# JGCRI/xanthos

Measured on AMD Instinct MI355X. Metric: cell-months/sec (pm_abcd_mrtm, 67,420 cells), higher is better.
Workload: dtype f64

## Files before the change

### xanthos_amd/csrc/xh_mrtm_wave_launch.hip

```cpp
#include <algorithm>
#include "xh_mrtm_wave_unit.h"
#undef A

namespace {

__global__ void k_mrtm_wave_args(WaveArgs a, WaveArgs *dst, uint4 *cnt, unsigned cnt_vec) {
    if (threadIdx.x == 0) *dst = a;
    if (threadIdx.x == 0 && a.months_ready)
        __hip_atomic_store(const_cast<unsigned *>(a.months_ready), a.ready_at_launch, __ATOMIC_RELAXED, __HIP_MEMORY_SCOPE_AGENT);
    for (unsigned i = threadIdx.x; i < cnt_vec; i += blockDim.x) cnt[i] = make_uint4(0u, 0u, 0u, 0u);
}

}

int wave_launch(xh_ctx *ctx, FlowPlan *fp, const FlowSched &s, const FlowIO &io, hipStream_t st, unsigned **place) {
    if (!fp || fp->n_units == 0) return XH_OK;
    if (!fp->skew_ok || fp->max_imports > 8 * SK_R || fp->max_exports > 8 * SK_R || s.ntmin < fp->skew_lmax + 2 * GROUP) {
        if (xh_flow_debug())
            fprintf(stderr, "time-skewed kernel not used: skew_ok %d, imports %d, outlets %d, shortest month %d sub-steps, largest lag %d\n",
                    (int)fp->skew_ok, fp->max_imports, fp->max_exports, s.ntmin, fp->skew_lmax);
        return XH_ERR_LIMIT;
    }
    {
        uint64_t limit = (uint64_t)1 << 32;
        if (const char *env = getenv("XH_WAVE_ROW_LIMIT")) limit = std::min<uint64_t>(limit, strtoull(env, nullptr, 10));
        const uint64_t stride = io.feed ? 128u : (uint64_t)s.nmonths * 8u;
        if ((uint64_t)(fp->max_cell + 1) * stride > limit || (io.feed && (int64_t)fp->max_cell >= io.feed->ncell)) {
            if (xh_flow_debug())
                fprintf(stderr, "round-3 time-skewed kernel not used: %d rows x %d months x 8 B exceed its 32-bit row offsets\n",
                        fp->max_cell + 1, s.nmonths);
            return XH_ERR_LIMIT;
        }
    }
    int rs = 2048;
    while (rs < 8 * CH + 4 * fp->skew_lmax || rs < 1024 + (2 * CH + 256) * fp->skew_span) rs *= 2;
    if (const char *env = getenv("XH_FLOW_RS")) {
        const int v = atoi(env);
        if (v >= 2048 && (v & (v - 1)) == 0) rs = v;
    }
    const size_t x_streams = (size_t)std::max(fp->n_edges, 1) * (size_t)rs * sizeof(v2d);
    if (x_streams + (size_t)rs * 16 > ((size_t)1 << 32)) return XH_ERR_LIMIT;
    const size_t x_cnt = ((size_t)(fp->n_edges + fp->n_units + PLACE_WORDS) * sizeof(unsigned) + 255) & ~size_t(255);
    const size_t x_rec0 = ((size_t)(s.nit + 3) * sizeof(MonthRec) + 255) & ~size_t(255);
    const size_t x_rec = x_rec0 + (((size_t)(s.nit + 2) * sizeof(FinRec) + 255) & ~size_t(255));
    if (x_streams + x_cnt + x_rec > fp->x_bytes) {
        if (fp->d_x) {
            XH_HIP(ctx, hipStreamSynchronize(st));
            XH_HIP(ctx, hipFree(fp->d_x));
            fp->d_x = nullptr;
        }
        XH_HIP(ctx, hipMalloc(&fp->d_x, x_streams + x_cnt + x_rec));
        fp->x_bytes = x_streams + x_cnt + x_rec;
        fp->rec_key = 0;
    }
    unsigned *cnt = reinterpret_cast<unsigned *>(static_cast<char *>(fp->d_x) + x_streams);
    MonthRec *d_rec = reinterpret_cast<MonthRec *>(static_cast<char *>(fp->d_x) + x_streams + x_cnt);
    FinRec *d_fin = reinterpret_cast<FinRec *>(static_cast<char *>(fp->d_x) + x_streams + x_cnt + x_rec0);
    const FlowFeed *feed = io.feed;
    auto q_off = [&](int m) -> long long {
        if (!feed) return (long long)m * 8;
        return (long long)(m >> 4) * feed->ncell * 128 + (long long)(m & 15) * 8;
    };
    uint64_t rec_key = XH_FNV_BASIS;
    {
        const long long lay[4] = {s.nit, s.total, feed ? (long long)feed->ncell : -1ll, (long long)(size_t)fp->d_x};
        rec_key = xh_fnv1a(rec_key, lay, sizeof(lay));
        rec_key = xh_fnv1a(rec_key, s.h_m, sizeof(int) * (size_t)s.nit);
        rec_key = xh_fnv1a(rec_key, s.h_nt, sizeof(int) * (size_t)s.nit);
        rec_key = xh_fnv1a(rec_key, s.h_g, sizeof(int) * (size_t)(s.nit + 1));
        rec_key = xh_fnv1a(rec_key, s.h_wr, (size_t)s.nit);
        rec_key = xh_fnv1a(rec_key, s.h_secs, sizeof(double) * (size_t)s.nit);
        if (rec_key == 0) rec_key = 1;
    }
    if (rec_key != fp->rec_key) {
        fp->rec_key = 0;
        fp->h_rec.assign((size_t)(s.nit + 3) * sizeof(MonthRec), 0);
        MonthRec *h = reinterpret_cast<MonthRec *>(fp->h_rec.data());
        for (int it = 0; it < s.nit; ++it) {
            h[it].m = s.h_m[it];
            h[it].nt = s.h_nt[it];
            h[it].g = s.h_g[it];
            h[it].write = s.h_wr[it];
            h[it].secs = s.h_secs[it];
            h[it].q_off = q_off(s.h_m[it]);
        }
        h[s.nit].g = s.total;
        fp->h_fin.assign((size_t)(s.nit + 2) * sizeof(FinRec), 0);
        FinRec *hf = reinterpret_cast<FinRec *>(fp->h_fin.data());
        for (int it = 0; it <= s.nit; ++it) {
            if (it >= 1) {
                hf[it].m_prev_w = h[it - 1].m | (h[it - 1].write ? FIN_WRITE : 0);
                hf[it].nt_prev = h[it - 1].nt;
            }
            hf[it].nt_prev = std::max(hf[it].nt_prev, 1);
            hf[it].secs_next1 = it + 1 < s.nit ? h[it + 1].secs : 1.0;
            hf[it].m_next2 = it + 2 < s.nit ? h[it + 2].m : 0;
            hf[it].q_off_next2 = q_off(hf[it].m_next2);
            hf[it].g_next1 = it + 1 <= s.nit ? h[it + 1].g : s.total;
        }
        hf[s.nit + 1].nt_prev = 1;
        hf[s.nit + 1].secs_next1 = 1.0;
        XH_HIP(ctx, hipMemcpyAsync(d_rec, h, fp->h_rec.size(), hipMemcpyHostToDevice, st));
        XH_HIP(ctx, hipMemcpyAsync(d_fin, hf, fp->h_fin.size(), hipMemcpyHostToDevice, st));
        fp->rec_key = rec_key;
    }

    const int cus = ctx->prop.multiProcessorCount > 0 ? ctx->prop.multiProcessorCount : 256;
    const void *kernel = fp->rsum ? wave_rsum_kernel() : wave_exact_kernel();
    const size_t lds_static = (size_t)RING * NSLOT * sizeof(v2d) + LANES * sizeof(uint2) + 2 * LANES * sizeof(unsigned) +
                              LANES * sizeof(double) + 64 +
                              (fp->rsum ? 2 * LANES * sizeof(unsigned) + LANES * sizeof(double) : 0);
    int n_excl = 0;
    if (fp->rsum && fp->n_special >= 0 && fp->n_pair_units > 0 && xh_env_on("XH_RSUM_EXCL", true))
        n_excl = std::min(fp->n_pair_units, 0xffff);
    int n_wg = 0, resident = 0;
    size_t lds = 0;
    {
        n_wg = fp->n_units + cus;
        if (n_wg > 8 * cus) n_wg = std::max(fp->n_units, 8 * cus);
        {
            const char *env = getenv("XH_FLOW_SPARE");
            if (env) n_wg = fp->n_units + std::max(atoi(env), 0);
        }
        const int per_cu = (n_wg + cus - 1) / cus + 3;
        const size_t share = ((size_t)(160 * 1024) / (size_t)per_cu) & ~size_t(1023);
        lds = share > lds_static + 1024 ? share - lds_static : 0;
        XH_HIP(ctx, hipFuncSetAttribute(kernel, hipFuncAttributeMaxDynamicSharedMemorySize, (int)lds));
        XH_HIP(ctx, hipOccupancyMaxActiveBlocksPerMultiprocessor(&resident, kernel, LANES, lds));
        if ((int64_t)(resident - 1) * cus < n_wg || n_wg > 8 * cus) return XH_ERR_LIMIT;
    }

    WaveArgs a;
    a.cell_of_slot = static_cast<const int *>(fp->d_cell_of_slot.p);
    a.lag = static_cast<const int *>(fp->d_lag.p);
    a.ghost_lag = static_cast<const int *>(fp->d_ghost_lag.p);
    a.export_edge = static_cast<const int *>(fp->d_export_edge.p);
    a.ghost_edge = static_cast<const int *>(fp->d_ghost_edge.p);
    a.edge_cons_unit = static_cast<const int *>(fp->d_edge_cons_unit.p);
    a.ent2 = static_cast<const unsigned *>(fp->d_ent2.p);
    a.eprev = static_cast<const unsigned *>(fp->d_eprev.p);
    a.unit_p = static_cast<const int *>(fp->d_unit_p.p);
    a.unit_order = static_cast<const int *>(fp->d_unit_order.p);
    a.n_units = fp->n_units;
    a.unit_lmax = static_cast<const int *>(fp->d_unit_lmax.p);
    a.unit_glmax = static_cast<const int *>(fp->d_unit_glmax.p);
    a.total_slots = (int64_t)fp->n_units * LANES;
    a.nmonths = s.nmonths;
    a.nit = s.nit;
    a.total = s.total;
    a.odd_ok = s.nt_even ? 0 : 1;
    a.rec = d_rec;
    a.fin = d_fin;
    a.lane_flags = static_cast<const unsigned char *>(fp->d_lane_flags.p);
    a.dt = s.dt;
    a.dtinv = 1.0 / s.dt;
    a.flow_dist = io.flow_dist;
    a.velocity = io.velocity;
    a.area = io.area;
    a.runoff = feed ? feed->q_staged : io.runoff;
    a.q_row_stride = feed ? 128u : (unsigned)s.nmonths * 8u;
    a.ready_at_launch = feed ? feed->ready_at_launch : UINT_MAX;
    a.months_ready = feed ? feed->months_ready : nullptr;
    a.place_epoch = feed ? feed->place_epoch : nullptr;
    a.epoch = feed ? feed->epoch : 0u;
    a.n_excl = n_excl;
    a.fenced = xh_env_on("XH_ROUTE_FENCED", false) ? 1 : 0;
    a.S0 = io.S0;
    a.chs = io.chs;
    a.avg = io.avg;
    a.S_end = io.S_end;
    a.F_end = io.F_end;
    a.xbuf = static_cast<char *>(fp->d_x);
    a.xbytes = (unsigned)x_streams;
    a.ring_mask_b = (unsigned)rs * 16u - 1u;
    a.rs = rs;
    a.ready = cnt;
    a.done = cnt + fp->n_edges;
    a.place = cnt + fp->n_edges + fp->n_units;
    *place = a.place;
    unsigned *fault = nullptr;
    int rc = xh_fault_word(ctx, &fault);
    if (rc) return rc;
    a.fault = fault;
    if (s.test_fault) XH_HIP(ctx, hipMemsetD32Async(reinterpret_cast<hipDeviceptr_t>(fault), (int)FAULT_TEST, 1, st));
    a.stats = nullptr;
    {
        const char *env = getenv("XH_FLOW_STATS");
        if (env && env[0] == '1') {
            if (!fp->d_stats) XH_HIP(ctx, hipMalloc(reinterpret_cast<void **>(&fp->d_stats), (size_t)fp->n_units * 48));
            a.stats = fp->d_stats;
        }
    }
    a.fold_cell = static_cast<const int *>(fp->d_fold_cell.p);
    if (!fp->d_skew_args) XH_HIP(ctx, hipMalloc(&fp->d_skew_args, sizeof(WaveArgs) + 256));
    hipLaunchKernelGGL(k_mrtm_wave_args, dim3(1), dim3(256), 0, st, a, static_cast<WaveArgs *>(fp->d_skew_args),
                       reinterpret_cast<uint4 *>(cnt), (unsigned)(x_cnt / sizeof(uint4)));
    {
        const WaveArgs *d_args = static_cast<const WaveArgs *>(fp->d_skew_args);
        void *kargs[] = {&d_args};
        XH_HIP(ctx, hipLaunchKernel(kernel, dim3((unsigned)n_wg), dim3(LANES), kargs, lds, st));
    }
    XH_HIP(ctx, hipGetLastError());
    return XH_OK;
}
```

### xanthos_amd/csrc/xh_mrtm_wave_unit.h

```cpp
#pragma once
#include <algorithm>
#include <climits>
#include <cstdlib>
#include <type_traits>

#include "xh_mrtm_flow.h"

namespace {


constexpr int LANES = 64;
constexpr int SK_P = 4;
#ifndef XH_WAVE_MIDZONE
#define XH_WAVE_MIDZONE 1
#endif
#ifndef XH_WAVE_BMOV
#define XH_WAVE_BMOV 1
#endif
constexpr int NSLOT = 2 * LANES + 1;
constexpr int RING = 8;
constexpr int GROUP = 16;
constexpr int SK_R = 2;
#ifndef XH_WAVE_CH
#define XH_WAVE_CH 256
#endif
constexpr int CH = XH_WAVE_CH;
constexpr unsigned FAULT_DATA_WAIT = 1, FAULT_RING_WAIT = 2, FAULT_PLACE_WAIT = 3, FAULT_GUARD = XH_FAULT_GUARD;
constexpr unsigned FAULT_TEST = 99;
constexpr int PLACE_KEYS = 16 * 8 * 2 * 16 * 4;

constexpr int PLACE_WORDS = 16 + PLACE_KEYS + PLACE_KEYS / 4;

struct MonthRec {
    int m, nt, g, write;
    double secs;
    long long q_off;
};
static_assert(sizeof(MonthRec) == 32, "MonthRec is read with one s_load_dwordx8");

struct FinRec {
    int m_prev_w, nt_prev;
    int m_next2;
    int g_next1;
    double secs_next1;
    long long q_off_next2;
};
constexpr int FIN_WRITE = 1 << 30;
static_assert(sizeof(FinRec) == 32, "FinRec is read with one s_load_dwordx8");

struct WaveArgs {
    const int *cell_of_slot, *lag, *ghost_lag, *export_edge, *ghost_edge, *edge_cons_unit;
    const unsigned *ent2;
    const unsigned *eprev;
    const int *unit_p, *unit_lmax, *unit_glmax;
    const unsigned char *lane_flags;
    int64_t total_slots;
    int nmonths, nit, total;
    const int *unit_order;
    unsigned *place;
    int n_units;
    int odd_ok;
    const MonthRec *rec;
    const FinRec *fin;
    double dt, dtinv;
    const double *flow_dist, *velocity, *area, *runoff, *S0;
    double *chs, *avg, *S_end, *F_end;
    unsigned q_row_stride;
    unsigned ready_at_launch;
    const unsigned *months_ready;
    unsigned *place_epoch;
    unsigned epoch;
    int n_excl;
    int fenced;
    char *xbuf;
    unsigned xbytes;
    unsigned ring_mask_b;
    int rs;
    unsigned *ready;
    unsigned *done;
    unsigned *fault;
    unsigned long long *stats;
    const int *fold_cell;
};

__device__ __forceinline__ unsigned ld_relaxed(const unsigned *p) {
    return __hip_atomic_load(p, __ATOMIC_RELAXED, __HIP_MEMORY_SCOPE_AGENT);
}

constexpr unsigned long long SPIN_LIMIT_TICKS = 500000000ull;

__device__ __forceinline__ bool wave_wait_ge(bool need, const unsigned *p, unsigned target, unsigned &seen,
                                             unsigned *fault, unsigned code) {
    bool ok = !need || seen >= target;
    if (__all(ok)) return true;
    const unsigned long long t0 = __builtin_amdgcn_s_memrealtime();
    for (;;) {
        if (!ok) {
            seen = ld_relaxed(p);
            ok = seen >= target;
        }
        if (__all(ok)) return true;
        if (ld_relaxed(fault) != 0) return false;
        if (__builtin_amdgcn_s_memrealtime() - t0 > SPIN_LIMIT_TICKS) {
            __hip_atomic_store(fault, code, __ATOMIC_RELAXED, __HIP_MEMORY_SCOPE_AGENT);
            return false;
        }
        __builtin_amdgcn_s_sleep(4);
    }
}

typedef double v2d __attribute__((ext_vector_type(2)));
typedef unsigned v4u __attribute__((ext_vector_type(4)));
constexpr int AUX_SC1 = 16;
typedef __attribute__((address_space(3))) const char lds_cchar;
typedef __attribute__((address_space(3))) char lds_char;

typedef __attribute__((address_space(4))) const WaveArgs WaveArgsK;
template <class T>
__device__ __forceinline__ T xh_ldarg(__attribute__((address_space(4))) const T *p) {
    asm volatile("" : "+s"(p));
    return *p;
}
#define A(f) xh_ldarg(&ap->f)

template <bool ONE> struct Val;
template <> struct Val<false> {
    typedef v2d T;
    typedef __attribute__((address_space(3))) const v2d lds_c;
    typedef __attribute__((address_space(3))) v2d lds_m;
    static constexpr unsigned B = 16;
    static __device__ __forceinline__ T zero() { return v2d{0.0, 0.0}; }
};
template <> struct Val<true> {
    typedef double T;
    typedef __attribute__((address_space(3))) const double lds_c;
    typedef __attribute__((address_space(3))) double lds_m;
    static constexpr unsigned B = 8;
    static __device__ __forceinline__ T zero() { return 0.0; }
};

template <int PRE, int POST, int NG, bool CHAIN, bool RSUM = false, bool FOLD = false, int SGL = 0, int NXR = -1>
__device__ __forceinline__ void wave_unit(WaveArgsK *ap, char *lds_generic, uint2 *xtab,
                                          __attribute__((address_space(3))) unsigned *qstage,
                                          __attribute__((address_space(3))) double *fend, const int unit) {
    constexpr bool HAS_G = NG > 0;
    constexpr bool V8 = SGL == 1;
    typedef Val<V8> V;
    typedef typename V::T val_t;
    typedef typename V::lds_c lds_cv;
    typedef typename V::lds_m lds_mv;
    constexpr unsigned VB = V::B;
    constexpr unsigned SLOTB = NSLOT * VB;
    lds_char *lds0 = (lds_char *)lds_generic;
    const int lane = threadIdx.x;
    const int64_t slot = (int64_t)unit * LANES + lane;

    const int gc = A(cell_of_slot)[slot];
    const bool valid = gc >= 0;
    const int gc_safe = valid ? gc : 0;
    const unsigned row_off = (unsigned)gc_safe * A(q_row_stride);
    const double tauinv = valid ? A(velocity)[gc] / A(flow_dist)[gc] : 0.0;
    const double acoef = 1.0 - tauinv * A(dt);
    const double area = valid ? A(area)[gc] : 0.0;
    const double S0v = (valid && A(S0)) ? A(S0)[gc] : 0.0;
    auto ent_off = [](unsigned o) { return V8 ? o >> 1 : o; };
    static_assert(!RSUM || (PRE <= 1 && POST == 0), "reassociated form: one inflow entry");
    static_assert(!FOLD || (RSUM && NG == 0), "folded leaves: reassociated form, units without imports");
    static_assert(SGL == 0 || RSUM, "single-sum plans: reassociated form");
    const int gcL = FOLD ? A(fold_cell)[slot] : -1;
    const bool validL = FOLD && valid && gcL >= 0;
    const unsigned row_offL = (unsigned)(validL ? gcL : 0) * A(q_row_stride);
    const double tauL = validL ? A(velocity)[gcL] / A(flow_dist)[gcL] : 0.0;
    const double acoefL = 1.0 - tauL * A(dt);
    const double areaL = validL ? A(area)[gcL] : 0.0;
    const double S0L = (validL && A(S0)) ? A(S0)[gcL] : 0.0;
    double SL = 0.0, favgL = 0.0, erlL = 0.0, erlL_n = 0.0, snapSL = 0.0, snapAL = 0.0, FL = 0.0;
    constexpr double FOLD_EPS = 1e-6;
    unsigned gfold = (validL && !(tauL * A(dt) <= 1.0 - 1.0 / 1048576.0 && tauL >= 0.0 && S0L >= 0.0)) ? 1u : 0u;
    constexpr double SGL_EPS = 1e-6;
    constexpr double SGL_XEPS = 1e-10;
    unsigned gsgl = 0;
    bool xlane = false;
    double fmin_seen = 0.0;
    if (SGL != 0) {
        const unsigned lf = A(lane_flags)[slot];
        xlane = valid && (lf & 2u) != 0;
        gsgl = (valid && (!(tauinv >= 0.0) || (!(tauinv * A(dt) <= 1.0 - 1.0 / 1048576.0) && !(lf & 1u)) || S0v < 0.0)) ? 1u : 0u;
    }
    constexpr int PRE_N = PRE > 0 ? PRE : 1, POST_N = POST > 0 ? POST : 1;
    lds_cchar *epre[PRE_N], *epost[POST_N];
#pragma unroll
    for (int w = 0; w < PRE; ++w) epre[w] = lds0 + ent_off(A(ent2)[(int64_t)w * A(total_slots) + slot]);
#pragma unroll
    for (int w = 0; w < POST; ++w) epost[w] = lds0 + ent_off(A(ent2)[(int64_t)(SK_P + w) * A(total_slots) + slot]);
    lds_cchar *eprv = lds0 + (CHAIN ? ent_off(A(eprev)[slot]) : 0u);
    lds_mv *own = (lds_mv *)lds0 + lane;
    const int xedge = A(export_edge)[slot];
    const int gedge = A(ghost_edge)[slot];
    const bool has_x = xedge >= 0, has_g = gedge >= 0;
    const unsigned long long xmask = __ballot(has_x), gmask = __ballot(has_g);
    const int nx_out = __popcll(xmask), ng = __popcll(gmask);
    static_assert(NXR >= -1 && NXR <= 1, "outlet rounds known at compile time: none or one");
    const bool any_x = NXR < 0 ? xmask != 0 : NXR > 0, any_g = HAS_G;
    const int lmax = A(unit_lmax)[unit], glmax = A(unit_glmax)[unit];
    const int lag_g = has_g ? A(ghost_lag)[slot] : 0;
    const unsigned *ready_p = A(ready) + (has_g ? gedge : 0);
    const unsigned *done_p = A(done) + (has_x ? A(edge_cons_unit)[xedge] : 0);
    const unsigned maskb = A(ring_mask_b);
    const unsigned oob = ~maskb;
    const __amdgpu_buffer_rsrc_t xr = __builtin_amdgcn_make_buffer_rsrc(A(xbuf), 0, (int)A(xbytes), 0x00020000);
    const int total = A(total), nit = A(nit);
    const bool odd_ok = A(odd_ok) != 0;

    if (has_x) xtab[__popcll(xmask & ((1ull << lane) - 1ull))] = make_uint2((unsigned)lane, (unsigned)xedge);
    const int sub = lane & 7, grp = lane >> 3;
    const bool x2 = NXR < 0 && nx_out > 8;
    unsigned gfull[SK_R], xbyte[SK_R];
    lds_mv *gdst[SK_R];
    lds_cv *xsrc[SK_R];
#pragma unroll
    for (int r = 0; r < SK_R; ++r) {
        const int k = r * 8 + grp;
        const bool gon = k < ng, xon = k < nx_out;
        const int ge = gon ? A(ghost_edge)[(int64_t)unit * LANES + k] : 0;
        const int gl = gon ? A(ghost_lag)[(int64_t)unit * LANES + k] : 0;
        gfull[r] = gon ? ((unsigned)ge * (maskb + 1u)) | (((unsigned)(sub - gl) * 16u) & maskb) : oob;
        gdst[r] = (lds_mv *)(lds0 + sub * SLOTB) + LANES + (k & 63);
        const uint2 t = xon ? xtab[k] : make_uint2((unsigned)lane, 0u);
        xbyte[r] = xon ? t.y * (maskb + 1u) + (unsigned)sub * 16u : oob;
        xsrc[r] = (lds_cv *)(lds0 + sub * SLOTB) + t.x;
    }
#pragma unroll
    for (int k = 0; k < RING; ++k) {
        own[k * NSLOT] = V::zero();
        own[k * NSLOT + LANES] = V::zero();
        if (lane == 0) own[k * NSLOT + 2 * LANES] = V::zero();
    }

    const double dt = A(dt), dtinv = A(dtinv);
    double S = 0.0, F = 0.0, favg = 0.0, erl = 0.0;
    double snapS = 0.0, snapA = 0.0;
    int nx = A(lag)[slot];
    const double *p_runoff = A(runoff);
    double *p_chs = A(chs), *p_avg = A(avg);
    typedef __attribute__((address_space(4))) const MonthRec MonthRecK;
    MonthRecK *p_rec = (MonthRecK *)A(rec);
    typedef __attribute__((address_space(4))) const FinRec FinRecK;
    FinRecK *p_fin = (FinRecK *)A(fin);
    auto ld_fin = [&](int i) {
        FinRec r;
        r.m_prev_w = p_fin[i].m_prev_w;
        r.nt_prev = p_fin[i].nt_prev;
        r.m_next2 = p_fin[i].m_next2;
        r.g_next1 = p_fin[i].g_next1;
        r.secs_next1 = p_fin[i].secs_next1;
        r.q_off_next2 = p_fin[i].q_off_next2;
        return r;
    };
    FinRec fc = ld_fin(0);
    auto ld_rec = [&](int i) {
        MonthRec r;
        r.m = p_rec[i].m;
        r.nt = p_rec[i].nt;
        r.g = p_rec[i].g;
        r.write = p_rec[i].write;
        r.secs = p_rec[i].secs;
        r.q_off = p_rec[i].q_off;
        return r;
    };
    const int nmo = A(nmonths);
    const unsigned q_lds = (unsigned)(size_t)qstage;
    auto runoff_fetch = [&](long long q_off) {
        const char *src = reinterpret_cast<const char *>(p_runoff) + q_off + (size_t)row_off;
        unsigned keep;
        asm volatile("s_mov_b32 %0, m0\n\ts_mov_b32 m0, %2\n\tglobal_load_lds_dword %1, off\n\ts_add_u32 m0, m0, 252\n\t"
                     "global_load_lds_dword %1, off offset:4\n\ts_mov_b32 m0, %0"
                     : "=&s"(keep)
                     : "v"(src), "s"(q_lds)
                     : "memory");
        if (FOLD) {
            const char *srcL = reinterpret_cast<const char *>(p_runoff) + q_off + (size_t)row_offL;
            asm volatile("s_mov_b32 %0, m0\n\ts_mov_b32 m0, %2\n\tglobal_load_lds_dword %1, off\n\ts_add_u32 m0, m0, 252\n\t"
                         "global_load_lds_dword %1, off offset:4\n\ts_mov_b32 m0, %0"
                         : "=&s"(keep)
                         : "v"(srcL), "s"(q_lds + 2u * LANES * 4u)
                         : "memory");
        }
    };
    auto runoff_take = [&]() {
        if (any_x || any_g) asm volatile("s_waitcnt vmcnt(4)" ::: "memory");
        else asm volatile("s_waitcnt vmcnt(0)" ::: "memory");
        const unsigned lo = qstage[lane], hi = qstage[LANES + lane];
        return __hiloint2double((int)hi, (int)lo);
    };
    double erl_n = 0.0;
    {
        const MonthRec r0 = ld_rec(0), r1 = ld_rec(1);
        auto ld_q = [&](long long q_off) {
            return *reinterpret_cast<const double *>(reinterpret_cast<const char *>(p_runoff) + q_off + (size_t)row_off);
        };
        const double q0 = ld_q(r0.q_off);
        erl_n = ((valid ? q0 : 0.0) * area) * 1000.0 / r0.secs;
        if (RSUM) erl_n *= A(dt);
        if (SGL != 0) gsgl |= (erl_n < -SGL_EPS) ? 2u : 0u;
        if (FOLD) {
            const double q0L = *reinterpret_cast<const double *>(reinterpret_cast<const char *>(p_runoff) + r0.q_off + (size_t)row_offL);
            erlL_n = (((validL ? q0L : 0.0) * areaL) * 1000.0 / r0.secs) * A(dt);
        }
        if (nit > 1) runoff_fetch(r1.q_off);
    }
    constexpr int OB = 4;
    double ob_s[OB], ob_a[OB];
    double ob_sL[FOLD ? OB : 1], ob_aL[FOLD ? OB : 1];
#pragma unroll
    for (int j = 0; j < OB; ++j) ob_s[j] = ob_a[j] = 0.0;
#pragma unroll
    for (int j = 0; j < (FOLD ? OB : 1); ++j) ob_sL[j] = ob_aL[j] = 0.0;
    bool alive = true;
    unsigned mready = A(ready_at_launch);
    auto wait_months = [&](unsigned need) {
        const unsigned *p = A(months_ready);
        if (!p) return true;
        const unsigned long long t0 = __builtin_amdgcn_s_memrealtime();
        for (;;) {
            unsigned v = 0;
            if (lane == 0) v = __hip_atomic_fetch_add(const_cast<unsigned *>(p), 0u, __ATOMIC_RELAXED, __HIP_MEMORY_SCOPE_AGENT);
            v = (unsigned)__builtin_amdgcn_readfirstlane((int)v);
            if (v >= need) {
                mready = v;
                return true;
            }
            if (ld_relaxed(A(fault)) != 0) return false;
            if (__builtin_amdgcn_s_memrealtime() - t0 > SPIN_LIMIT_TICKS) {
                __hip_atomic_store(A(fault), FAULT_DATA_WAIT, __ATOMIC_RELAXED, __HIP_MEMORY_SCOPE_AGENT);
                return false;
            }
            __builtin_amdgcn_s_sleep(16);
        }
    };
    unsigned long long cyc_wait_data = 0, cyc_wait_ring = 0, zone_groups = 0;
    const unsigned long long cyc_begin = __builtin_amdgcn_s_memtime();
    const unsigned long long rt_begin = __builtin_amdgcn_s_memrealtime();

    unsigned seen_ready = 0, seen_done = 0, pend_ready = 0, pend_done = 0;
    auto load_async = [&](const unsigned *q) {
        unsigned v;
        asm volatile("global_load_dword %0, %1, off sc1" : "=v"(v) : "v"(q) : "memory");
        return v;
    };
    auto check = [&](int n) {
        const unsigned long long w0 = __builtin_amdgcn_s_memtime();
        asm volatile("s_waitcnt vmcnt(8)" : "+v"(pend_ready), "+v"(pend_done) : : "memory");
        asm volatile("s_waitcnt vmcnt(0)" ::: "memory");
        if (SGL == 2) gsgl |= (xlane && fmin_seen < -SGL_XEPS) ? 4u : 0u;
        if ((FOLD && __any(gfold != 0)) || (SGL != 0 && __any(gsgl != 0))) {
            __hip_atomic_store(A(fault), FAULT_GUARD, __ATOMIC_RELAXED, __HIP_MEMORY_SCOPE_AGENT);
            alive = false;
        }
        const bool fenced = A(fenced) == 1;
        if (any_x) {
            const int pub = min(max(n - RING - lmax, 0), total);
            if (fenced) __builtin_amdgcn_fence(__ATOMIC_RELEASE, "agent");
            if (has_x) __hip_atomic_store(A(ready) + xedge, (unsigned)pub, __ATOMIC_RELAXED, __HIP_MEMORY_SCOPE_AGENT);
            const int need = n + CH - lmax - A(rs);
            seen_done = max(seen_done, pend_done);
            if (need > 0 && alive)
                alive = wave_wait_ge(has_x, done_p, (unsigned)min(need, total), seen_done, A(fault), FAULT_RING_WAIT);
        }
        const unsigned long long w1 = __builtin_amdgcn_s_memtime();
        if (any_g && alive) {
            if (lane == 0)
                __hip_atomic_store(A(done) + unit, (unsigned)min(max(n - glmax, 0), total), __ATOMIC_RELAXED,
                                   __HIP_MEMORY_SCOPE_AGENT);
            const int need = min(total, n + CH + GROUP - lag_g);
            seen_ready = max(seen_ready, pend_ready);
            alive = wave_wait_ge(has_g && need > 0, ready_p, (unsigned)max(need, 0), seen_ready, A(fault), FAULT_DATA_WAIT);
            if (fenced) __builtin_amdgcn_fence(__ATOMIC_ACQUIRE, "agent");
            asm volatile("" ::: "memory");
        }
        if (any_x) pend_done = load_async(done_p);
        if (any_g) pend_ready = load_async(ready_p);
        cyc_wait_ring += w1 - w0;
        cyc_wait_data += __builtin_amdgcn_s_memtime() - w1;
    };

    auto finalize = [&](int it) {
        const FinRec f = fc;
        fc = ld_fin(it + 1 <= nit ? it + 1 : nit + 1);
        if (it + 1 < nit) {
            const double qn = runoff_take();
            erl_n = ((valid ? qn : 0.0) * area) * 1000.0 / f.secs_next1;
            if (RSUM) erl_n *= dt;
            if (SGL != 0) gsgl |= (erl_n < -SGL_EPS) ? 2u : 0u;
            if (FOLD) {
                const unsigned lo = qstage[2 * LANES + lane], hi = qstage[3 * LANES + lane];
                const double qnL = __hiloint2double((int)hi, (int)lo);
                erlL_n = (((validL ? qnL : 0.0) * areaL) * 1000.0 / f.secs_next1) * dt;
            }
        }
        if (it >= 1) {
            const int m = f.m_prev_w & (FIN_WRITE - 1);
            const bool write_prev = (f.m_prev_w & FIN_WRITE) != 0;
#pragma unroll
            for (int j = 0; j < OB - 1; ++j) {
                ob_s[j] = ob_s[j + 1];
                ob_a[j] = ob_a[j + 1];
            }
            ob_s[OB - 1] = snapS;
            ob_a[OB - 1] = snapA / (double)f.nt_prev;
            if (FOLD) {
#pragma unroll
                for (int j = 0; j < OB - 1; ++j) {
                    ob_sL[j] = ob_sL[j + 1];
                    ob_aL[j] = ob_aL[j + 1];
                }
                ob_sL[OB - 1] = snapSL;
                ob_aL[OB - 1] = snapAL / (double)f.nt_prev;
                gfold |= (snapSL < -FOLD_EPS) ? 2u : 0u;
                if (write_prev && validL) {
                    if ((m & (OB - 1)) == OB - 1) {
                        const int64_t o = (int64_t)gcL * nmo + (m - (OB - 1));
#pragma unroll
                        for (int j = 0; j < OB; j += 2) {
                            if (p_chs) *reinterpret_cast<v2d *>(p_chs + o + j) = v2d{ob_sL[j], ob_sL[j + 1]};
                            if (p_avg) *reinterpret_cast<v2d *>(p_avg + o + j) = v2d{ob_aL[j], ob_aL[j + 1]};
                        }
                    } else if (m == nmo - 1) {
                        const int r = (m & (OB - 1)) + 1;
                        const int64_t o = (int64_t)gcL * nmo + (m + 1 - r);
#pragma unroll
                        for (int j = 0; j < OB; ++j)
                            if (j >= OB - r) {
                                if (p_chs) p_chs[o + j - (OB - r)] = ob_sL[j];
                                if (p_avg) p_avg[o + j - (OB - r)] = ob_aL[j];
                            }
                    }
                }
            }
            if (write_prev && valid) {
                if ((m & (OB - 1)) == OB - 1) {
                    const int64_t o = (int64_t)gc * nmo + (m - (OB - 1));
#pragma unroll
                    for (int j = 0; j < OB; j += 2) {
                        if (p_chs) *reinterpret_cast<v2d *>(p_chs + o + j) = v2d{ob_s[j], ob_s[j + 1]};
                        if (p_avg) *reinterpret_cast<v2d *>(p_avg + o + j) = v2d{ob_a[j], ob_a[j + 1]};
                    }
                } else if (m == nmo - 1) {
                    const int r = (m & (OB - 1)) + 1;
                    const int64_t o = (int64_t)gc * nmo + (m + 1 - r);
#pragma unroll
                    for (int j = 0; j < OB; ++j)
                        if (j >= OB - r) {
                            if (p_chs) p_chs[o + j - (OB - r)] = ob_s[j];
                            if (p_avg) p_avg[o + j - (OB - r)] = ob_a[j];
                        }
                }
            }
        }
        if (it + 2 < nit) {
            if ((unsigned)f.m_next2 >= mready) alive = wait_months((unsigned)f.m_next2 + 1u);
            if (alive) runoff_fetch(f.q_off_next2);
        }
        return f.g_next1;
    };

    val_t va[2][PRE_N], vb[2][POST_N], vr[2];
    v4u gbuf[2][SK_R];
#pragma unroll
    for (int q = 0; q < 2; ++q) {
#pragma unroll
        for (int w = 0; w < PRE; ++w) va[q][w] = V::zero();
#pragma unroll
        for (int w = 0; w < POST; ++w) vb[q][w] = V::zero();
        vr[q] = V::zero();
    }
    auto import_load = [&](int r) {
        const v4u v = __builtin_amdgcn_raw_buffer_load_b128(xr, gfull[r], 0, AUX_SC1);
        gfull[r] = (gfull[r] & ~maskb) | ((gfull[r] + RING * 16u) & maskb);
        return v;
    };
    auto import_drop = [&](int r, const v4u u) {
        if (SGL == 1) {
            typedef unsigned v2u __attribute__((ext_vector_type(2)));
            *reinterpret_cast<__attribute__((address_space(3))) v2u *>(gdst[r]) = v2u{u.z, u.w};
        } else {
            *reinterpret_cast<__attribute__((address_space(3))) v4u *>(gdst[r]) = u;
        }
    };
    val_t xb[SK_R];
#pragma unroll
    for (int r = 0; r < SK_R; ++r) {
        xb[r] = V::zero();
    }
    auto block_io = [&](const int b) {
        if (HAS_G) {
#pragma unroll
            for (int r = 0; r < NG; ++r) {
                import_drop(r, gbuf[b][r]);
                gbuf[b][r] = import_load(r);
            }
        }
        if (any_x) {
            xb[0] = *xsrc[0];
            if (x2) xb[1] = *xsrc[1];
        }
    };
    auto store_pair = [&](const val_t v, unsigned voff, unsigned soff) {
        v2d p;
        if constexpr (SGL == 1) p = v2d{v, v};
        else p = v;
        __builtin_amdgcn_raw_buffer_store_b128(__builtin_bit_cast(v4u, p), xr, voff, soff, AUX_SC1);
    };
    auto block_store = [&](int m0) {
        if (any_x) {
            const unsigned xpos = ((unsigned)(m0 - RING - lmax) * 16u) & maskb;
            store_pair(xb[0], xbyte[0], xpos);
            if (x2) store_pair(xb[1], xbyte[1], xpos);
        }
    };

    check(0);
#pragma unroll
    for (int r = 0; r < SK_R; ++r) gbuf[0][r] = r < NG ? import_load(r) : v4u{0u, 0u, 0u, 0u};
#pragma unroll
    for (int r = 0; r < SK_R; ++r) gbuf[1][r] = r < NG ? import_load(r) : v4u{0u, 0u, 0u, 0u};

    const int N = (total + lmax + 1 + GROUP - 1) & ~(GROUP - 1);
    int itz = 0, gz = 0;
    int itf = 0, nf = (lmax + 1 + GROUP - 1) & ~(GROUP - 1);
    int ntz = nit > 0 ? p_rec[0].nt : 0;

    auto substep = [&](auto zone_c, auto mid_c, const int n, const int j, const int edge, const int rel) {
        constexpr bool MID = decltype(mid_c)::value;
        if (decltype(zone_c)::value && ((j & 1) == 0 || (!MID && odd_ok))) {
            const bool c = rel == j;
#if XH_WAVE_BMOV
            {
                const unsigned long long cm = __ballot(c);
                unsigned long long sv;
                asm volatile("s_and_saveexec_b64 %[sv], %[cm]\n\tv_mov_b64 %[ss], %[s]\n\tv_mov_b64 %[sa], %[fa]\n\t"
                             "v_mov_b64 %[fa], 0\n\tv_mov_b64 %[e], %[en]\n\ts_mov_b64 exec, %[sv]"
                             : [ss] "+v"(snapS), [sa] "+v"(snapA), [fa] "+v"(favg), [e] "+v"(erl), [sv] "=&s"(sv)
                             : [s] "v"(S), [en] "v"(erl_n), [cm] "s"(cm)
                             : "scc");
            }
#else
            snapS = c ? S : snapS;
            snapA = c ? favg : snapA;

            favg = c ? 0.0 : favg;
            erl = c ? erl_n : erl;
#endif
            if (FOLD) {
                snapSL = c ? SL : snapSL;
                snapAL = c ? favgL : snapAL;
                favgL = c ? 0.0 : favgL;
                erlL = c ? erlL_n : erlL;
            }
            if (!MID) {
                if (edge == 1) S = c ? S0v : S;
                if (FOLD && edge == 1) SL = c ? S0L : SL;
                if (edge == 2) {
                    if (c) fend[lane] = F;
                    if (FOLD && c) fend[LANES + lane] = FL;
                }
            }
        }
        __builtin_amdgcn_sched_barrier(0);
        val_t(&ac)[PRE_N] = va[j & 1], (&bc)[POST_N] = vb[j & 1], (&an)[PRE_N] = va[(j & 1) ^ 1], (&bn)[POST_N] = vb[(j & 1) ^ 1];
        const val_t rc = vr[j & 1];
        const unsigned so = (unsigned)((j + RING - 1) & (RING - 1)) * SLOTB;
        if (CHAIN) vr[(j & 1) ^ 1] = *(lds_cv *)(eprv + so);
#pragma unroll
        for (int w = 0; w < PRE; ++w) an[w] = *(lds_cv *)(epre[w] + so);
#pragma unroll
        for (int w = 0; w < POST; ++w) bn[w] = *(lds_cv *)(epost[w] + so);
        __builtin_amdgcn_sched_barrier(0);
        __builtin_amdgcn_s_waitcnt(0xC07F | ((PRE + POST + (CHAIN ? 1 : 0) + 1) << 8));
        __builtin_amdgcn_sched_barrier(0);
        if ((j & (RING - 1)) == 0) block_io(j / RING);
        if ((j & (RING - 1)) == 1) block_store(n + j - 1);
        const double F0 = S * tauinv;
        if constexpr (RSUM) {
            double base = __builtin_fma(S, acoef, erl);
            if (FOLD) {
                FL = SL * tauL;
                SL = __builtin_fma(SL, acoefL, erlL);
                favgL += FL;
                base = __builtin_fma(FL, dt, base);
            }
            if constexpr (SGL == 1) {
                const double S1 = PRE ? __builtin_fma(ac[0], dt, base) : base;
                const double m = __builtin_fmin(S1, 0.0);
                const double f2 = __builtin_fma(m, dtinv, F0);
                own[(j & (RING - 1)) * NSLOT] = CHAIN ? rc + f2 : f2;
                S = S1 - m;
                F = f2;
                favg += f2;
            } else {
            const double S1 = PRE ? __builtin_fma(ac[0].x, dt, base) : base;
            const double S2 = PRE ? __builtin_fma(ac[0].y, dt, base) : base;
            const bool sx = S1 < 0.0;
            const double f2 = __builtin_fma(__builtin_fmin(S1, 0.0), dtinv, F0);
            own[(j & (RING - 1)) * NSLOT] = CHAIN ? v2d{rc.x + F0, rc.y + f2} : v2d{F0, f2};
            double Sn = S2;
            asm volatile("" : "+v"(Sn));
            S = sx ? 0.0 : Sn;
            F = f2;
            favg += f2;
            if (SGL == 2) fmin_seen = __builtin_fmin(fmin_seen, f2);
            }
        } else {
            double s1 = 0.0, s2 = 0.0;
#pragma unroll
            for (int w = 0; w < PRE; ++w) {
                s1 += ac[w].x;
                s2 += ac[w].y;
            }
            s1 -= F0;
#pragma unroll
            for (int w = 0; w < POST; ++w) s1 += bc[w].x;
            const double dsdt = s1 + erl;
            const bool sx = (dsdt * dt) < (-S);
            const double f2 = sx ? (dsdt + F0) + S * dtinv : F0;
            own[(j & (RING - 1)) * NSLOT] = CHAIN ? v2d{rc.x + F0, rc.y + f2} : v2d{F0, f2};
            s2 -= f2;
#pragma unroll
            for (int w = 0; w < POST; ++w) s2 += bc[w].y;
            const double dsdt2 = s2 + erl;
            double Sn = S + dsdt2 * dt;
            asm volatile("" : "+v"(Sn));
            S = sx ? 0.0 : Sn;
            F = f2;
            favg += f2;
        }
    };

#ifdef XH_WAVE_PROFILE
    unsigned long long prof_zone = 0, prof_fin = 0, prof_t = __builtin_amdgcn_s_memtime();
#define PROF_MARK(acc)                                                  \
    {                                                                   \
        const unsigned long long now_ = __builtin_amdgcn_s_memtime();   \
        acc += now_ - prof_t;                                           \
        prof_t = now_;                                                  \
    }
    unsigned long long prof_plain = 0;
#else
#define PROF_MARK(acc)
#endif
    auto housekeeping = [&](int n) {
        if (n > 0 && (n & (CH - 1)) == 0) check(n);
        if (alive && n == nf) {
            const int g_next = finalize(itf);
            ++itf;
            nf = itf <= nit ? ((g_next + lmax + 1 + GROUP - 1) & ~(GROUP - 1)) : INT_MAX;
        }
        PROF_MARK(prof_fin)
    };
    int n = 0;
    while (n < N && alive) {
        if (itz <= nit && n + GROUP > gz && n <= gz + lmax) {
            const int edge = itz == 0 ? 1 : (itz == nit ? 2 : 0);
            auto zone_run = [&](auto mid_c) {
                do {
                    housekeeping(n);
                    if (!alive) break;
                    ++zone_groups;
                    const int rel = nx - n;
#pragma unroll
                    for (int j = 0; j < GROUP; ++j) substep(std::true_type(), mid_c, n, j, edge, rel);
                    n += GROUP;
                    PROF_MARK(prof_zone)
                } while (n <= gz + lmax && n < N);
            };
#if XH_WAVE_MIDZONE
            if (edge == 0 && !odd_ok) zone_run(std::true_type());
            else zone_run(std::false_type());
#else
            zone_run(std::false_type());
#endif
            if (alive) {
                nx = itz < nit ? nx + ntz : INT_MAX;
                ++itz;
                gz = p_rec[itz <= nit ? itz : nit].g;
                if (itz > nit) gz = INT_MAX;
                ntz = p_rec[itz <= nit ? itz : nit].nt;
            }
        } else {
            const int n_end = itz <= nit ? min(N, gz & ~(GROUP - 1)) : N;
            do {
                housekeeping(n);
                if (!alive) break;
#pragma unroll
                for (int j = 0; j < GROUP; ++j) substep(std::false_type(), std::false_type(), n, j, 0, 0);
                n += GROUP;
                PROF_MARK(prof_plain)
            } while (n < n_end);
        }
    }
    if (alive) {
        while (itf <= nit) finalize(itf++);
        if (SGL == 2) gsgl |= (xlane && fmin_seen < -SGL_XEPS) ? 4u : 0u;
        if ((FOLD && __any(gfold != 0)) || (SGL != 0 && __any(gsgl != 0))) {
            __hip_atomic_store(A(fault), FAULT_GUARD, __ATOMIC_RELAXED, __HIP_MEMORY_SCOPE_AGENT);
            alive = false;
        }
    }
    if (alive) {
        if (any_x) {
            const unsigned xpos = ((unsigned)(N - RING - lmax) * 16u) & maskb;
            store_pair(*xsrc[0], xbyte[0], xpos);
            if (x2) store_pair(*xsrc[1], xbyte[1], xpos);
            asm volatile("s_waitcnt vmcnt(0)" ::: "memory");
            if (A(fenced) == 1) __builtin_amdgcn_fence(__ATOMIC_RELEASE, "agent");
            if (has_x) __hip_atomic_store(A(ready) + xedge, (unsigned)total, __ATOMIC_RELAXED, __HIP_MEMORY_SCOPE_AGENT);
        }
        if (any_g && lane == 0)
            __hip_atomic_store(A(done) + unit, (unsigned)total, __ATOMIC_RELAXED, __HIP_MEMORY_SCOPE_AGENT);
        if (valid) {
            if (A(S_end)) A(S_end)[gc] = snapS;
            if (A(F_end)) A(F_end)[gc] = fend[lane];
        }
        if (validL) {
            if (A(S_end)) A(S_end)[gcL] = snapSL;
            if (A(F_end)) A(F_end)[gcL] = fend[LANES + lane];
        }
    }
    const bool guard_set = __any((gfold | gsgl) != 0);
    if (A(stats) && lane == 0) {
        unsigned long long *st = A(stats) + (int64_t)unit * 6;
        const unsigned long long cyc = __builtin_amdgcn_s_memtime() - cyc_begin;
        st[0] = cyc - cyc_wait_data - cyc_wait_ring;
        st[1] = cyc;
        st[2] = __builtin_amdgcn_s_memrealtime() - rt_begin;
        const unsigned hw = __builtin_amdgcn_s_getreg((4) | (0 << 6) | (31 << 11));
        const unsigned xcc = __builtin_amdgcn_s_getreg((20) | (0 << 6) | (3 << 11));
        st[3] = (unsigned long long)((PRE + POST + (CHAIN ? 1 : 0) + 1) & 15) | (any_g ? 16u : 0u) | (any_x ? 32u : 0u) |
                (V8 ? 64u : 0u) | (guard_set ? 128u : 0u) | ((unsigned long long)hw << 8) | ((unsigned long long)(xcc & 15u) << 40) |
                (zone_groups << 44);
        st[4] = cyc_wait_data;
        st[5] = cyc_wait_ring;
#ifdef XH_WAVE_PROFILE
        st[0] = prof_plain;
        st[4] = prof_zone;
        st[5] = prof_fin;
#endif
    }
}


__device__ __forceinline__ int wave_claim(WaveArgsK *ap, int *unit_sh_p, int *prio_sh_p) {
    int &unit_sh = *unit_sh_p, &prio_sh = *prio_sh_p;
    if (threadIdx.x == 0) {
        prio_sh = 0;
        unsigned *pl = A(place);
        const unsigned hw = __builtin_amdgcn_s_getreg((4) | (0 << 6) | (31 << 11));
        const unsigned xcc = __builtin_amdgcn_s_getreg((20) | (0 << 6) | (3 << 11)) & 15u;
        const unsigned key = ((((xcc * 8u + ((hw >> 13) & 7u)) * 2u + ((hw >> 12) & 1u)) * 16u + ((hw >> 8) & 15u)) * 4u) +
                             ((hw >> 4) & 3u);
        unsigned *pl_cu = pl + 16 + PLACE_KEYS + (key >> 2);
        const int n_units = A(n_units);
        const unsigned n_wg = gridDim.x;
        unsigned *fault = A(fault);
        auto wait_for = [&](unsigned *word, unsigned target) {
            const unsigned long long t0 = __builtin_amdgcn_s_memrealtime();
            while (__hip_atomic_load(word, __ATOMIC_ACQUIRE, __HIP_MEMORY_SCOPE_AGENT) < target) {
                if (ld_relaxed(fault) != 0 || __builtin_amdgcn_s_memrealtime() - t0 > SPIN_LIMIT_TICKS) {
                    __hip_atomic_store(fault, FAULT_PLACE_WAIT, __ATOMIC_RELAXED, __HIP_MEMORY_SCOPE_AGENT);
                    return false;
                }
                __builtin_amdgcn_s_sleep(8);
            }
            return true;
        };
        auto add = [&](int word) { return __hip_atomic_fetch_add(pl + word, 1u, __ATOMIC_RELAXED, __HIP_MEMORY_SCOPE_AGENT); };
        const unsigned rank = __hip_atomic_fetch_add(pl + 16 + key, 1u, __ATOMIC_RELAXED, __HIP_MEMORY_SCOPE_AGENT) & 0xffffu;
        bool leader = false;
        unsigned cu_rank = 0;
        if (rank == 0) {
            add(2);
            cu_rank = __hip_atomic_fetch_add(pl_cu, 1u, __ATOMIC_RELAXED, __HIP_MEMORY_SCOPE_AGENT) & 0xffffu;
            leader = cu_rank == 0u;
            if (leader) add(9);
        } else if (rank == 1) {
            add(1);
        }
        const unsigned registered = __hip_atomic_fetch_add(pl + 0, 1u, __ATOMIC_RELEASE, __HIP_MEMORY_SCOPE_AGENT);
        if (registered + 1u == n_wg && A(place_epoch))
            __hip_atomic_store(A(place_epoch), A(epoch), __ATOMIC_RELAXED, __HIP_MEMORY_SCOPE_AGENT);
        int idx = -1;
        if (wait_for(pl + 0, n_wg)) {
            const int firsts = (int)ld_relaxed(pl + 2), seconds = (int)ld_relaxed(pl + 1), leaders = (int)ld_relaxed(pl + 9);
            const int n_excl = A(n_excl);
            int ncu = min(n_excl, leaders);
            ncu = max(min(ncu, (seconds - max(n_units - firsts, 0)) / 7), 0);
            bool excl_cu = false;
            int displaced = 0, claimed = 0;
            bool ok = true;
            if (ncu > 0) {
                if (leader) {
                    if ((int)add(10) < ncu) {
                        const int cnt = (int)(ld_relaxed(pl_cu) & 0xffffu);
                        const int base = (int)add(13);
                        if (base < n_excl) {
                            __hip_atomic_fetch_or(pl_cu, 0x10000u, __ATOMIC_RELAXED, __HIP_MEMORY_SCOPE_AGENT);
                            __hip_atomic_fetch_add(pl + 11, (unsigned)(cnt - 1), __ATOMIC_RELAXED, __HIP_MEMORY_SCOPE_AGENT);
                            idx = n_units - 1 - base;
                        }
                    }
                    __hip_atomic_fetch_add(pl + 12, 1u, __ATOMIC_RELEASE, __HIP_MEMORY_SCOPE_AGENT);
                }
                ok = wait_for(pl + 12, (unsigned)leaders);
                excl_cu = (ld_relaxed(pl_cu) & 0x10000u) != 0;
                displaced = (int)ld_relaxed(pl + 11);
                claimed = min((int)ld_relaxed(pl + 13), n_excl);
            }
            const int nx = claimed;
            const int firsts_eff = firsts - displaced;
            const int need2 = max(n_units - firsts_eff, 0);
            if (idx >= 0 || !ok) {
            } else if (rank >= 2) {
                idx = -2;
            } else if (rank == 1) {
                const int t = excl_cu ? INT_MAX : (int)add(3);
                if (t < need2) __hip_atomic_fetch_or(pl + 16 + key, 0x10000u, __ATOMIC_RELAXED, __HIP_MEMORY_SCOPE_AGENT);
                __hip_atomic_fetch_add(pl + 4, 1u, __ATOMIC_RELEASE, __HIP_MEMORY_SCOPE_AGENT);
                idx = t < need2 ? t : -2;
                if (t < need2) prio_sh = 1;
            } else if (excl_cu) {
                idx = -2;
            } else if (wait_for(pl + 4, (unsigned)seconds)) {
                const bool shared = (ld_relaxed(pl + 16 + key) & 0x10000u) != 0;
                if (firsts_eff > n_units && (int)add(7) >= n_units - nx) {
                    idx = -2;
                } else if (shared) {
                    idx = need2 + (int)add(5);
                    prio_sh = 3;
                } else {
                    idx = 2 * need2 + (int)add(6);
                }
                if (idx >= n_units - nx) idx = -1;
            }
            if (idx >= n_units) idx = -1;
        }
        if (idx == -1) __hip_atomic_store(fault, FAULT_PLACE_WAIT, __ATOMIC_RELAXED, __HIP_MEMORY_SCOPE_AGENT);
        unit_sh = idx >= 0 ? A(unit_order)[idx] : -1;
    }
    __syncthreads();
    return unit_sh;
}

}
```

Measured before the change: 3.152 billion.

## Restructure wave main loop and precompute per-month scale factors in FinRec

Moves the per-month record fill into a shared helper and extends FinRec to 64 bytes with a precomputed runoff scale (1000*dt/secs), the reciprocal of the previous sub-step count, and the current sub-step count. The kernel uses these to replace divisions with multiplies in the rsum path. It also merges zone advancement into finalize so the two counters become one. The main loop is restructured so the periodic check and finalize run only at chunk boundaries instead of every group. In exchange, FinRec loads are larger and the rsum path can round slightly differently from the original division.

After: 3.224 billion (median of 6 runs). 1.02x the previous value.

```diff
diff --git a/xanthos_amd/csrc/xh_mrtm_rec.h b/xanthos_amd/csrc/xh_mrtm_rec.h
--- /dev/null
+++ b/xanthos_amd/csrc/xh_mrtm_rec.h
@@ -0,0 +1,56 @@
+#pragma once
+#include <algorithm>
+#include <cstddef>
+
+struct MonthRec {
+    int m, nt, g, write;
+    double secs;
+    long long q_off;
+};
+static_assert(sizeof(MonthRec) == 32, "MonthRec is read with one s_load_dwordx8");
+
+struct FinRec {
+    int m_prev_w, nt_prev;
+    int m_next2;
+    int g_next1;
+    double secs_next1;
+    long long q_off_next2;
+    double erl_scale_next1;
+    double inv_nt_prev;
+    int nt_cur;
+    int pad_[3];
+};
+constexpr int FIN_WRITE = 1 << 30;
+static_assert(sizeof(FinRec) == 64, "FinRec is one 64-byte line");
+
+template <class QOff>
+inline void wave_fill_records(int nit, int total, double dt, const int *m, const int *nt, const int *g, const unsigned char *wr,
+                              const double *secs, QOff q_off, MonthRec *h, FinRec *hf) {
+    for (int it = 0; it < nit; ++it) {
+        h[it].m = m[it];
+        h[it].nt = nt[it];
+        h[it].g = g[it];
+        h[it].write = wr[it];
+        h[it].secs = secs[it];
+        h[it].q_off = q_off(m[it]);
+    }
+    h[nit].g = total;
+    for (int it = 0; it <= nit; ++it) {
+        if (it >= 1) {
+            hf[it].m_prev_w = h[it - 1].m | (h[it - 1].write ? FIN_WRITE : 0);
+            hf[it].nt_prev = h[it - 1].nt;
+        }
+        hf[it].nt_prev = std::max(hf[it].nt_prev, 1);
+        hf[it].secs_next1 = it + 1 < nit ? h[it + 1].secs : 1.0;
+        hf[it].m_next2 = it + 2 < nit ? h[it + 2].m : 0;
+        hf[it].q_off_next2 = q_off(hf[it].m_next2);
+        hf[it].g_next1 = it + 1 <= nit ? h[it + 1].g : total;
+        hf[it].erl_scale_next1 = 1000.0 * dt / hf[it].secs_next1;
+        hf[it].inv_nt_prev = 1.0 / (double)hf[it].nt_prev;
+        hf[it].nt_cur = it < nit ? h[it].nt : 0;
+    }
+    hf[nit + 1].nt_prev = 1;
+    hf[nit + 1].secs_next1 = 1.0;
+    hf[nit + 1].erl_scale_next1 = 1000.0 * dt;
+    hf[nit + 1].inv_nt_prev = 1.0;
+}
diff --git a/xanthos_amd/csrc/xh_mrtm_wave_launch.hip b/xanthos_amd/csrc/xh_mrtm_wave_launch.hip
--- a/xanthos_amd/csrc/xh_mrtm_wave_launch.hip
+++ b/xanthos_amd/csrc/xh_mrtm_wave_launch.hip
@@ -70,36 +70,16 @@
         rec_key = xh_fnv1a(rec_key, s.h_g, sizeof(int) * (size_t)(s.nit + 1));
         rec_key = xh_fnv1a(rec_key, s.h_wr, (size_t)s.nit);
         rec_key = xh_fnv1a(rec_key, s.h_secs, sizeof(double) * (size_t)s.nit);
+        rec_key = xh_fnv1a(rec_key, &s.dt, sizeof(double));
         if (rec_key == 0) rec_key = 1;
     }
     if (rec_key != fp->rec_key) {
         fp->rec_key = 0;
         fp->h_rec.assign((size_t)(s.nit + 3) * sizeof(MonthRec), 0);
         MonthRec *h = reinterpret_cast<MonthRec *>(fp->h_rec.data());
-        for (int it = 0; it < s.nit; ++it) {
-            h[it].m = s.h_m[it];
-            h[it].nt = s.h_nt[it];
-            h[it].g = s.h_g[it];
-            h[it].write = s.h_wr[it];
-            h[it].secs = s.h_secs[it];
-            h[it].q_off = q_off(s.h_m[it]);
-        }
-        h[s.nit].g = s.total;
         fp->h_fin.assign((size_t)(s.nit + 2) * sizeof(FinRec), 0);
         FinRec *hf = reinterpret_cast<FinRec *>(fp->h_fin.data());
-        for (int it = 0; it <= s.nit; ++it) {
-            if (it >= 1) {
-                hf[it].m_prev_w = h[it - 1].m | (h[it - 1].write ? FIN_WRITE : 0);
-                hf[it].nt_prev = h[it - 1].nt;
-            }
-            hf[it].nt_prev = std::max(hf[it].nt_prev, 1);
-            hf[it].secs_next1 = it + 1 < s.nit ? h[it + 1].secs : 1.0;
-            hf[it].m_next2 = it + 2 < s.nit ? h[it + 2].m : 0;
-            hf[it].q_off_next2 = q_off(hf[it].m_next2);
-            hf[it].g_next1 = it + 1 <= s.nit ? h[it + 1].g : s.total;
-        }
-        hf[s.nit + 1].nt_prev = 1;
-        hf[s.nit + 1].secs_next1 = 1.0;
+        wave_fill_records(s.nit, s.total, s.dt, s.h_m, s.h_nt, s.h_g, s.h_wr, s.h_secs, q_off, h, hf);
         XH_HIP(ctx, hipMemcpyAsync(d_rec, h, fp->h_rec.size(), hipMemcpyHostToDevice, st));
         XH_HIP(ctx, hipMemcpyAsync(d_fin, hf, fp->h_fin.size(), hipMemcpyHostToDevice, st));
         fp->rec_key = rec_key;
diff --git a/xanthos_amd/csrc/xh_mrtm_wave_unit.h b/xanthos_amd/csrc/xh_mrtm_wave_unit.h
--- a/xanthos_amd/csrc/xh_mrtm_wave_unit.h
+++ b/xanthos_amd/csrc/xh_mrtm_wave_unit.h
@@ -5,6 +5,7 @@
 #include <type_traits>
 
 #include "xh_mrtm_flow.h"
+#include "xh_mrtm_rec.h"
 
 namespace {
 
@@ -30,23 +31,6 @@
 constexpr int PLACE_KEYS = 16 * 8 * 2 * 16 * 4;
 
 constexpr int PLACE_WORDS = 16 + PLACE_KEYS + PLACE_KEYS / 4;
-
-struct MonthRec {
-    int m, nt, g, write;
-    double secs;
-    long long q_off;
-};
-static_assert(sizeof(MonthRec) == 32, "MonthRec is read with one s_load_dwordx8");
-
-struct FinRec {
-    int m_prev_w, nt_prev;
-    int m_next2;
-    int g_next1;
-    double secs_next1;
-    long long q_off_next2;
-};
-constexpr int FIN_WRITE = 1 << 30;
-static_assert(sizeof(FinRec) == 32, "FinRec is read with one s_load_dwordx8");
 
 struct WaveArgs {
     const int *cell_of_slot, *lag, *ghost_lag, *export_edge, *ghost_edge, *edge_cons_unit;
@@ -248,13 +232,19 @@
     typedef __attribute__((address_space(4))) const FinRec FinRecK;
     FinRecK *p_fin = (FinRecK *)A(fin);
     auto ld_fin = [&](int i) {
-        FinRec r;
+        FinRec r = {};
         r.m_prev_w = p_fin[i].m_prev_w;
-        r.nt_prev = p_fin[i].nt_prev;
         r.m_next2 = p_fin[i].m_next2;
         r.g_next1 = p_fin[i].g_next1;
-        r.secs_next1 = p_fin[i].secs_next1;
         r.q_off_next2 = p_fin[i].q_off_next2;
+        r.nt_cur = p_fin[i].nt_cur;
+        if constexpr (RSUM) {
+            r.erl_scale_next1 = p_fin[i].erl_scale_next1;
+            r.inv_nt_prev = p_fin[i].inv_nt_prev;
+        } else {
+            r.nt_prev = p_fin[i].nt_prev;
+            r.secs_next1 = p_fin[i].secs_next1;
+        }
         return r;
     };
     FinRec fc = ld_fin(0);
@@ -300,13 +290,17 @@
             return *reinterpret_cast<const double *>(reinterpret_cast<const char *>(p_runoff) + q_off + (size_t)row_off);
         };
         const double q0 = ld_q(r0.q_off);
-        erl_n = ((valid ? q0 : 0.0) * area) * 1000.0 / r0.secs;
-        if (RSUM) erl_n *= A(dt);
+        if constexpr (RSUM) {
+            const double scale0 = 1000.0 * A(dt) / r0.secs;
+            erl_n = ((valid ? q0 : 0.0) * area) * scale0;
+            if (FOLD) {
+                const double q0L = *reinterpret_cast<const double *>(reinterpret_cast<const char *>(p_runoff) + r0.q_off + (size_t)row_offL);
+                erlL_n = ((validL ? q0L : 0.0) * areaL) * scale0;
+            }
+        } else {
+            erl_n = ((valid ? q0 : 0.0) * area) * 1000.0 / r0.secs;
+        }
         if (SGL != 0) gsgl |= (erl_n < -SGL_EPS) ? 2u : 0u;
-        if (FOLD) {
-            const double q0L = *reinterpret_cast<const double *>(reinterpret_cast<const char *>(p_runoff) + r0.q_off + (size_t)row_offL);
-            erlL_n = (((validL ? q0L : 0.0) * areaL) * 1000.0 / r0.secs) * A(dt);
-        }
         if (nit > 1) runoff_fetch(r1.q_off);
     }
     constexpr int OB = 4;
@@ -389,13 +383,13 @@
         fc = ld_fin(it + 1 <= nit ? it + 1 : nit + 1);
         if (it + 1 < nit) {
             const double qn = runoff_take();
-            erl_n = ((valid ? qn : 0.0) * area) * 1000.0 / f.secs_next1;
-            if (RSUM) erl_n *= dt;
+            if constexpr (RSUM) erl_n = ((valid ? qn : 0.0) * area) * f.erl_scale_next1;
+            else erl_n = ((valid ? qn : 0.0) * area) * 1000.0 / f.secs_next1;
             if (SGL != 0) gsgl |= (erl_n < -SGL_EPS) ? 2u : 0u;
             if (FOLD) {
                 const unsigned lo = qstage[2 * LANES + lane], hi = qstage[3 * LANES + lane];
                 const double qnL = __hiloint2double((int)hi, (int)lo);
-                erlL_n = (((validL ? qnL : 0.0) * areaL) * 1000.0 / f.secs_next1) * dt;
+                erlL_n = ((validL ? qnL : 0.0) * areaL) * f.erl_scale_next1;
             }
         }
         if (it >= 1) {
@@ -407,7 +401,8 @@
                 ob_a[j] = ob_a[j + 1];
             }
             ob_s[OB - 1] = snapS;
-            ob_a[OB - 1] = snapA / (double)f.nt_prev;
+            if constexpr (RSUM) ob_a[OB - 1] = snapA * f.inv_nt_prev;
+            else ob_a[OB - 1] = snapA / (double)f.nt_prev;
             if (FOLD) {
 #pragma unroll
                 for (int j = 0; j < OB - 1; ++j) {
@@ -415,7 +410,7 @@
                     ob_aL[j] = ob_aL[j + 1];
                 }
                 ob_sL[OB - 1] = snapSL;
-                ob_aL[OB - 1] = snapAL / (double)f.nt_prev;
+                ob_aL[OB - 1] = snapAL * f.inv_nt_prev;
                 gfold |= (snapSL < -FOLD_EPS) ? 2u : 0u;
                 if (write_prev && validL) {
                     if ((m & (OB - 1)) == OB - 1) {
@@ -461,7 +456,6 @@
             if ((unsigned)f.m_next2 >= mready) alive = wait_months((unsigned)f.m_next2 + 1u);
             if (alive) runoff_fetch(f.q_off_next2);
         }
-        return f.g_next1;
     };
 
     val_t va[2][PRE_N], vb[2][POST_N], vr[2];
@@ -527,8 +521,7 @@
 
     const int N = (total + lmax + 1 + GROUP - 1) & ~(GROUP - 1);
     int itz = 0, gz = 0;
-    int itf = 0, nf = (lmax + 1 + GROUP - 1) & ~(GROUP - 1);
-    int ntz = nit > 0 ? p_rec[0].nt : 0;
+    int nf = (lmax + 1 + GROUP - 1) & ~(GROUP - 1);
 
     auto substep = [&](auto zone_c, auto mid_c, const int n, const int j, const int edge, const int rel) {
         constexpr bool MID = decltype(mid_c)::value;
@@ -637,7 +630,7 @@
     };
 
 #ifdef XH_WAVE_PROFILE
-    unsigned long long prof_zone = 0, prof_fin = 0, prof_t = __builtin_amdgcn_s_memtime();
+    unsigned long long prof_zone = 0, prof_fin = 0, prof_check = 0, prof_zx = 0, prof_hk = 0, prof_t = __builtin_amdgcn_s_memtime();
 #define PROF_MARK(acc)                                                  \
     {                                                                   \
         const unsigned long long now_ = __builtin_amdgcn_s_memtime();   \
@@ -648,30 +641,37 @@
 #else
 #define PROF_MARK(acc)
 #endif
-    auto housekeeping = [&](int n) {
-        if (n > 0 && (n & (CH - 1)) == 0) check(n);
+    int n = 0;
+    for (;;) {
+        PROF_MARK(prof_hk)
+        if (n > 0 && n < N && (n & (CH - 1)) == 0) {
+            check(n);
+            PROF_MARK(prof_check)
+        }
         if (alive && n == nf) {
-            const int g_next = finalize(itf);
-            ++itf;
-            nf = itf <= nit ? ((g_next + lmax + 1 + GROUP - 1) & ~(GROUP - 1)) : INT_MAX;
-        }
-        PROF_MARK(prof_fin)
-    };
-    int n = 0;
-    while (n < N && alive) {
-        if (itz <= nit && n + GROUP > gz && n <= gz + lmax) {
+            nx = itz < nit ? nx + fc.nt_cur : INT_MAX;
+            gz = itz < nit ? fc.g_next1 : INT_MAX;
+            PROF_MARK(prof_zx)
+            finalize(itz);
+            ++itz;
+            nf = itz <= nit ? ((gz + lmax + 1 + GROUP - 1) & ~(GROUP - 1)) : INT_MAX;
+            PROF_MARK(prof_fin)
+        }
+        if (n >= N || !alive) break;
+        const int stop = min(N, (n | (CH - 1)) + 1);
+        PROF_MARK(prof_hk)
+        if (n + GROUP > gz) {
             const int edge = itz == 0 ? 1 : (itz == nit ? 2 : 0);
+            const int n_end = min(nf, stop);
             auto zone_run = [&](auto mid_c) {
                 do {
-                    housekeeping(n);
-                    if (!alive) break;
                     ++zone_groups;
                     const int rel = nx - n;
 #pragma unroll
                     for (int j = 0; j < GROUP; ++j) substep(std::true_type(), mid_c, n, j, edge, rel);
                     n += GROUP;
                     PROF_MARK(prof_zone)
-                } while (n <= gz + lmax && n < N);
+                } while (n < n_end);
             };
 #if XH_WAVE_MIDZONE
             if (edge == 0 && !odd_ok) zone_run(std::true_type());
@@ -679,18 +679,9 @@
 #else
             zone_run(std::false_type());
 #endif
-            if (alive) {
-                nx = itz < nit ? nx + ntz : INT_MAX;
-                ++itz;
-                gz = p_rec[itz <= nit ? itz : nit].g;
-                if (itz > nit) gz = INT_MAX;
-                ntz = p_rec[itz <= nit ? itz : nit].nt;
-            }
         } else {
-            const int n_end = itz <= nit ? min(N, gz & ~(GROUP - 1)) : N;
+            const int n_end = min(stop, gz & ~(GROUP - 1));
             do {
-                housekeeping(n);
-                if (!alive) break;
 #pragma unroll
                 for (int j = 0; j < GROUP; ++j) substep(std::false_type(), std::false_type(), n, j, 0, 0);
                 n += GROUP;
@@ -699,7 +690,6 @@
         }
     }
     if (alive) {
-        while (itf <= nit) finalize(itf++);
         if (SGL == 2) gsgl |= (xlane && fmin_seen < -SGL_XEPS) ? 4u : 0u;
         if ((FOLD && __any(gfold != 0)) || (SGL != 0 && __any(gsgl != 0))) {
             __hip_atomic_store(A(fault), FAULT_GUARD, __ATOMIC_RELAXED, __HIP_MEMORY_SCOPE_AGENT);
@@ -743,7 +733,10 @@
 #ifdef XH_WAVE_PROFILE
         st[0] = prof_plain;
         st[4] = prof_zone;
-        st[5] = prof_fin;
+        st[1] = (cyc & 0xffffffffull) | ((cyc_wait_data + cyc_wait_ring) << 32);
+        st[2] = (prof_check << 32) | (prof_hk & 0xffffffffull);
+        st[5] = (prof_fin << 32) | (prof_zx & 0xffffffffull);
+        if (FOLD) st[3] |= 1ull << 63;
 #endif
     }
 }
```
